# KarelPeeters/kZero

Measured on AMD Instinct MI355X. Metric: self-play NN evals/sec (node), Chess 20x256 ResNet b=256, 1/2/4/8 GPU, higher is better.
Workload: dtype f16; 1 GPU; chess-20x256 attention head, executor batch 256; engines_per_gpu=1, parallelism=dp1 (no collective)

## Files before the change

### kzero_amd/csrc/kz_tower.hip

```cpp
#include <cstdlib>
#include <type_traits>
#include <vector>

#include "kz_kernels.hpp"
#include "kz_launch.hpp"

namespace kz {

typedef _Float16 h16;
typedef h16 h16x8 __attribute__((ext_vector_type(8)));
typedef h16 h16x4 __attribute__((ext_vector_type(4)));
typedef float f32x4 __attribute__((ext_vector_type(4)));

namespace {

#include "kz_decode_dev.hpp"
#include "kz_encode_dev.hpp"

constexpr int C = 256;
constexpr int RS = C * 2 + 16;
constexpr int URS = 3 * C * 2 + 16;
constexpr int KSTEPS = 72;
constexpr int HEAD_KSTEPS = 5 * 8;
constexpr int POLICY = 1880, LOGIT_LD = 96;
constexpr int TOWER_PF_MAX = 8;

struct TowerDev {
    const h16 *x0;
    const uint4 *w_stem, *w_tower;
    const float *bias, *post_scale, *post_shift;
    h16 *y;
    int cin_p, batch, depth;
    PackedBoards in;
    const float *sh_w0, *sh_b0, *sh_w1, *sh_b1, *sh_w2, *sh_b2;
    const int32_t *att_idx;
    float *scalars, *policy;
    int *nonfinite_flag;
    int epoch;
    DecodeDev dec;
};

template <int I, int N, class F>
__device__ __forceinline__ void static_for(F &&f) {
    if constexpr (I < N) {
        f(std::integral_constant<int, I>{});
        static_for<I + 1, N>(f);
    }
}

template <int NB>
struct Layout {
    static constexpr int M = NB * 64;
    static constexpr int MT = M / 16;
    static constexpr bool LINE_TILES = NB == 2;
    static constexpr int BPAD = LINE_TILES ? 128 : 0;
    static constexpr int BOARD = 64 * RS + BPAD;
    static constexpr int TS = LINE_TILES ? 8 * RS : 16 * RS;
    static constexpr int IMG = NB * BOARD;
    static constexpr int X_OFF = 0;
    static constexpr int Y_OFF = IMG;
    static constexpr int Z_OFF = 2 * IMG;
    static_assert(Z_OFF % 256 == 0, "zero rows keep the slot pattern of the image rows");
    static constexpr int S_OFF = Z_OFF + 16 * RS;
    static constexpr int TOWER_BYTES = S_OFF + M * 64;
    static constexpr int U_OFF = Z_OFF;
    static constexpr int ACT_OFF = U_OFF + 16 * URS;
    static constexpr int HID_OFF = ACT_OFF + NB * 256 * 4;
    static constexpr int HEADS_BYTES = HID_OFF + NB * 32 * 4;
    static constexpr int LOG_OFF = Y_OFF;
    static constexpr int BYTES = TOWER_BYTES > HEADS_BYTES ? TOWER_BYTES : HEADS_BYTES;
    static_assert(NB * 64 * LOGIT_LD * 4 <= IMG, "logits fit the Y region");
    static constexpr int row_off(int b, int p) { return b * BOARD + p * RS; }
    static_assert(BYTES <= 160 * 1024, "LDS budget");
};

constexpr int SG_VALU = 0x2, SG_SALU = 0x4, SG_MFMA = 0x8, SG_VMEM_READ = 0x20, SG_DS_READ = 0x100;

template <int NB, bool HEADS, int PF, bool WIDE = false, bool PREV = false>
__global__ __launch_bounds__(256, 1) void kz_tower_resident(TowerDev a) {
    using L = Layout<NB>;
    constexpr int M = L::M, MT = L::MT;
    static_assert(PF <= TOWER_PF_MAX, "the refills past the end of the stream must land in its padding");
    extern __shared__ __attribute__((aligned(16))) unsigned char lds[];

    const int tid = threadIdx.x;
    const int wave = __builtin_amdgcn_readfirstlane(tid >> 6);
    const int lane = tid & 63;
    const int fr = lane & 15, kq = lane >> 4;
    const int board0 = blockIdx.x * NB;
    const int layers = 2 * a.depth;
    const int total_ksteps = layers * KSTEPS + (HEADS ? HEAD_KSTEPS : 0);
    const int bias_rows = layers + (HEADS ? 5 : 0);

    const uint4 *wp = a.w_tower + wave * 256 + lane;
    auto wload_prev = [&](int gk, int nt) __attribute__((always_inline)) { return wp[(size_t)gk * 1024 + nt * 64]; };
    typedef const __attribute__((address_space(1))) unsigned char *gptr;
    gptr wk = (gptr)a.w_tower + wave * 4096;
    const unsigned wlane = lane * 16;
    auto wload = [&](gptr k, int nt) __attribute__((always_inline)) {
        typedef unsigned u32x4 __attribute__((ext_vector_type(4)));
        return __builtin_bit_cast(uint4, *reinterpret_cast<const __attribute__((address_space(1))) u32x4 *>(k + wlane + nt * 1024));
    };
    uint4 wreg[PF][4];
#pragma unroll
    for (int s = 0; s < PF; s++) {
        const int g = s < total_ksteps ? s : total_ksteps - 1;
#pragma unroll
        for (int nt = 0; nt < 4; nt++) wreg[s][nt] = PREV ? wload_prev(g, nt) : wload(wk + s * 16384, nt);
    }
    wk += PF * 16384;
    int g = 0;
    auto ring_take = [&](int stage, h16x8 (&af)[4]) __attribute__((always_inline)) {
#pragma unroll
        for (int nt = 0; nt < 4; nt++) af[nt] = *reinterpret_cast<const h16x8 *>(&wreg[stage][nt]);
#ifndef KZ_TW_NO_WLOAD
        if constexpr (PREV) {
            const int gn = g + PF < total_ksteps ? g + PF : total_ksteps - 1;
#pragma unroll
            for (int nt = 0; nt < 4; nt++) wreg[stage][nt] = wload_prev(gn, nt);
        } else {
#pragma unroll
            for (int nt = 0; nt < 4; nt++) wreg[stage][nt] = wload(wk, nt);
        }
#endif
        wk += 16384;
        if constexpr (!PREV) asm("" : "+s"(wk));
    };

    const int sc = WIDE ? a.cin_p >> 5 : 1;
    const int stem_off = WIDE ? L::Y_OFF : L::S_OFF, srow = 64 * sc, spieces = 4 * sc;
    for (int id = tid; id < 16 * RS / 16; id += 256)
        *reinterpret_cast<uint4 *>(lds + L::Z_OFF + id * 16) = make_uint4(0, 0, 0, 0);
    for (int id = tid; id < M * spieces; id += 256) {
        const int row = WIDE ? id / spieces : id >> 2, c = id - row * spieces;
        const int board = board0 + (row >> 6);
        uint4 v = make_uint4(0, 0, 0, 0);
        if (board < a.batch) {
            if (a.in.bits) {
                h16x8 e;
#pragma unroll
                for (int j = 0; j < 8; j++) e[j] = (h16)encoded_plane(a.in, board, c * 8 + j, row & 63, 64);
                v = *reinterpret_cast<const uint4 *>(&e);
            } else {
                v = *reinterpret_cast<const uint4 *>(a.x0 + ((size_t)board0 * 64 + row) * a.cin_p + c * 8);
            }
        }
        *reinterpret_cast<uint4 *>(lds + stem_off + row * srow + c * 16) = v;
    }
    __syncthreads();

    f32x4 acc[4][MT];
    f32x4 bias_next[4];
    auto fetch_bias = [&](int row) __attribute__((always_inline)) {
        const int l = row <= bias_rows ? row : bias_rows;
#pragma unroll
        for (int nt = 0; nt < 4; nt++)
            bias_next[nt] = *reinterpret_cast<const f32x4 *>(a.bias + l * C + wave * 64 + nt * 16 + kq * 4);
    };
    auto init_acc = [&]() __attribute__((always_inline)) {
#pragma unroll
        for (int nt = 0; nt < 4; nt++)
#pragma unroll
            for (int mt = 0; mt < MT; mt++) acc[nt][mt] = bias_next[nt];
    };
    f32x4 post_s[4], post_t[4];
#pragma unroll
    for (int nt = 0; nt < 4; nt++) {
        post_s[nt] = f32x4{1.f, 1.f, 1.f, 1.f};
        post_t[nt] = f32x4{0.f, 0.f, 0.f, 0.f};
    }

    auto relu4 = [](f32x4 v) {
        typedef int i32x4 __attribute__((ext_vector_type(4)));
        i32x4 b = __builtin_bit_cast(i32x4, v);
#pragma unroll
        for (int j = 0; j < 4; j++) b[j] = b[j] > 0 ? b[j] : 0;
        return __builtin_bit_cast(f32x4, b);
    };
    auto to_h4 = [](f32x4 v) { return h16x4{(h16)v[0], (h16)v[1], (h16)v[2], (h16)v[3]}; };

    const int lane_row = L::LINE_TILES ? (fr >> 3) * L::BOARD + (fr & 7) * RS : fr * RS;
    const int epi_base = lane_row + (wave * 64 + kq * 4) * 2;
    auto epilogue = [&](int dst_off, auto relu, auto residual, auto post) __attribute__((always_inline)) {
#pragma unroll
        for (int nt = 0; nt < 4; nt++) {
            h16x4 rx[MT];
            if constexpr (decltype(residual)::value) {
#pragma unroll
                for (int mt = 0; mt < MT; mt++)
                    rx[mt] = *reinterpret_cast<const h16x4 *>(lds + L::X_OFF + epi_base + mt * L::TS + nt * 32);
            }
#pragma unroll
            for (int mt = 0; mt < MT; mt++) {
                const int off = epi_base + mt * L::TS + nt * 32;
                f32x4 v = acc[nt][mt];
                if constexpr (decltype(relu)::value) v = relu4(v);
                if constexpr (decltype(residual)::value) {
#pragma unroll
                    for (int j = 0; j < 4; j++) v[j] += (float)rx[mt][j];
                }
                if constexpr (decltype(post)::value) v = v * post_s[nt] + post_t[nt];
                *reinterpret_cast<h16x4 *>(lds + dst_off + off) = to_h4(v);
            }
        }
    };
    constexpr std::true_type YES{};
    constexpr std::false_type NO{};

    const bool x_is0 = (lane & 7) == 0, x_is7 = (lane & 7) == 7, yo_is0 = (lane & 8) == 0, yo_is1 = !yo_is0;
    auto tap_ok = [&](int mt, int dy, int dx) __attribute__((always_inline)) {
        const bool kill_x = (dx < 0 && x_is0) || (dx > 0 && x_is7);
        if constexpr (L::LINE_TILES) return !(kill_x || (dy < 0 && mt == 0) || (dy > 0 && mt == MT - 1));
        else return !(kill_x || ((mt & 3) == 0 && dy < 0 && yo_is0) || ((mt & 3) == 3 && dy > 0 && yo_is1));
    };

    fetch_bias(0);
    init_acc();
    fetch_bias(1);
    for (int ks = 0; ks < 9 * sc; ks++) {
        const int tap = WIDE ? ks / sc : ks, chunk = ks - tap * sc;
        const int dy = tap / 3 - 1, dx = tap % 3 - 1;
        h16x8 af[4];
#pragma unroll
        for (int nt = 0; nt < 4; nt++) {
            const uint4 t = a.w_stem[((ks * 4 + wave) * 4 + nt) * 64 + lane];
            af[nt] = *reinterpret_cast<const h16x8 *>(&t);
        }
#pragma unroll
        for (int mt = 0; mt < MT; mt++) {
            const bool ok = tap_ok(mt, dy, dx);
            const int p = L::LINE_TILES ? (fr >> 3) * 64 + mt * 8 + (fr & 7) : mt * 16 + fr;
            const int off = ok ? stem_off + (p + dy * 8 + dx) * srow + chunk * 64 + kq * 16 : L::Z_OFF + kq * 16;
            const h16x8 bf = *reinterpret_cast<const h16x8 *>(lds + off);
#pragma unroll
            for (int nt = 0; nt < 4; nt++)
                acc[nt][mt] = __builtin_amdgcn_mfma_f32_16x16x32_f16(af[nt], bf, acc[nt][mt], 0, 0, 0);
        }
    }
    epilogue(L::X_OFF, NO, NO, NO);
    __syncthreads();

    const int kq_off = 256 * (kq & 1) + 128 * (kq >> 1);
    const int frag_base = lane_row + kq_off;
    auto tap_rows = [&](int dy, int dx, int src_off, int (&T)[MT]) __attribute__((always_inline)) {
        const int shifted = frag_base + src_off + (dy * 8 + dx) * RS;
        const int zrow = L::Z_OFF + ((fr + dy * 8 + dx) & 15) * RS + kq_off;
        const int zrow_odd = L::LINE_TILES ? L::Z_OFF + ((fr + dy * 8 + dx + 8) & 15) * RS + kq_off : zrow;
        if constexpr (PREV) {
#pragma unroll
            for (int mt = 0; mt < MT; mt++) T[mt] = tap_ok(mt, dy, dx) ? shifted + mt * L::TS : ((mt & 1) ? zrow_odd : zrow);
        } else {
            int z0 = zrow, z1 = zrow_odd;
            asm("" : "+v"(z0), "+v"(z1));
            const bool kill_x = ((dx < 0) & x_is0) | ((dx > 0) & x_is7);
#pragma unroll
            for (int mt = 0; mt < MT; mt++) {
                bool kill = kill_x;
                if constexpr (!L::LINE_TILES) kill = kill_x | (((mt & 3) == 0) & (dy < 0) & yo_is0) | (((mt & 3) == 3) & (dy > 0) & yo_is1);
                T[mt] = kill ? ((mt & 1) ? z1 : z0) : shifted + mt * L::TS;
            }
        }
    };

    h16x8 bf[2][MT];
    constexpr auto tile_lo = [](int dy) { return L::LINE_TILES && dy < 0 ? 1 : 0; };
    constexpr auto tile_hi = [](int dy) { return L::LINE_TILES && dy > 0 ? MT - 1 : MT; };

    auto conv_plain = [&](auto ndy_tag, int src_off, int dx_lo, int dx_hi) __attribute__((always_inline)) {
        constexpr int NDY = decltype(ndy_tag)::value, DY0 = NDY == 3 ? -1 : 0;
        int T[NDY][MT], Tn[NDY][MT];
#pragma unroll
        for (int i = 0; i < NDY; i++) tap_rows(DY0 + i, dx_lo, src_off, T[i]);
#pragma unroll
        for (int mt = tile_lo(DY0); mt < tile_hi(DY0); mt++) bf[0][mt] = *reinterpret_cast<const h16x8 *>(lds + T[0][mt]);
#pragma nounroll
        for (int dx = dx_lo; dx < dx_hi; dx++) {
#pragma unroll
            for (int i = 0; i < NDY; i++) tap_rows(DY0 + i, dx + 1 < dx_hi ? dx + 1 : dx, src_off, Tn[i]);
            static_for<0, 8 * NDY>([&](auto s_tag) __attribute__((always_inline)) {
                constexpr int s = decltype(s_tag)::value, ch = s / NDY, i = s % NDY, dy = DY0 + i;
                constexpr int stage = s & (PF - 1), cur = s & 1, nxt = cur ^ 1;
                constexpr int lo = tile_lo(dy), hi = tile_hi(dy), nt_ = hi - lo;
                constexpr int in_ = (i + 1) % NDY, chn = i + 1 < NDY ? ch : ch + 1;
                constexpr int lon = tile_lo(DY0 + in_), hin = tile_hi(DY0 + in_), nr = hin - lon;
#ifndef KZ_TW_NO_DSREAD
#pragma unroll
                for (int mt = 0; mt < MT; mt++) {
                    if (mt >= lon && mt < hin)
                        bf[nxt][mt] = *reinterpret_cast<const h16x8 *>(lds + (chn < 8 ? T[in_][mt] + chn * 16 : Tn[in_][mt]));
                }
#endif
                h16x8 af[4];
                ring_take(stage, af);
#pragma unroll
                for (int nt = 0; nt < 4; nt++)
#pragma unroll
                    for (int mt = 0; mt < MT; mt++)
                        if (mt >= lo && mt < hi)
                            acc[nt][mt] = __builtin_amdgcn_mfma_f32_16x16x32_f16(af[nt], bf[cur][mt], acc[nt][mt], 0, 0, 0);
#pragma unroll
                for (int j = 0; j < 4; j++) {
                    __builtin_amdgcn_sched_group_barrier(SG_MFMA, 1, 0);
                    __builtin_amdgcn_sched_group_barrier(SG_VMEM_READ, 1, 0);
                }
#pragma unroll
                for (int j = 0; j < MT; j++) {
                    if (j < nr) {
                        __builtin_amdgcn_sched_group_barrier(SG_MFMA, 1, 0);
                        __builtin_amdgcn_sched_group_barrier(SG_DS_READ, 1, 0);
                    }
                }
                constexpr int n_free = 4 * nt_ - (nr + 4), n_alu = PREV || s != 0 ? 0 : n_free < 20 ? n_free : 20;
#pragma unroll
                for (int j = 0; j < 20; j++) {
                    if (j < n_alu) {
                        __builtin_amdgcn_sched_group_barrier(SG_MFMA, 1, 0);
                        __builtin_amdgcn_sched_group_barrier(SG_VALU | SG_SALU, 2, 0);
                    }
                }
                __builtin_amdgcn_sched_group_barrier(SG_MFMA, n_free - n_alu, 0);
                __builtin_amdgcn_sched_barrier(0);
                g++;
            });
#pragma unroll
            for (int i = 0; i < NDY; i++)
#pragma unroll
                for (int mt = 0; mt < MT; mt++) T[i][mt] = Tn[i][mt];
        }
    };

    auto conv_3x3_lines = [&](int src_off) __attribute__((always_inline)) {
        static_assert(!L::LINE_TILES || MT == 8, "one tile per board line");
        int T[MT], Tn[MT];
        tap_rows(0, -1, src_off, T);
#pragma unroll
        for (int mt = 0; mt < MT; mt++) bf[0][mt] = *reinterpret_cast<const h16x8 *>(lds + T[mt]);
#pragma nounroll
        for (int dx = -1; dx < 2; dx++) {
            tap_rows(0, dx < 1 ? dx + 1 : dx, src_off, Tn);
            static_for<0, 8>([&](auto ch_tag) __attribute__((always_inline)) {
                constexpr int ch = decltype(ch_tag)::value, cur = ch & 1, nxt = cur ^ 1;
#ifndef KZ_TW_NO_DSREAD
#pragma unroll
                for (int mt = 0; mt < MT; mt++)
                    bf[nxt][mt] = *reinterpret_cast<const h16x8 *>(lds + (ch < 7 ? T[mt] + (ch + 1) * 16 : Tn[mt]));
#endif
                static_for<0, 3>([&](auto i_tag) __attribute__((always_inline)) {
                    constexpr int i = decltype(i_tag)::value, dy = i - 1, stage = (ch * 3 + i) & (PF - 1);
                    constexpr int lo = tile_lo(dy), hi = tile_hi(dy), nt_ = hi - lo;
                    h16x8 af[4];
                    ring_take(stage, af);
#pragma unroll
                    for (int nt = 0; nt < 4; nt++)
#pragma unroll
                        for (int mt = 0; mt < MT; mt++)
                            if (mt >= lo && mt < hi)
                                acc[nt][mt] = __builtin_amdgcn_mfma_f32_16x16x32_f16(af[nt], bf[cur][mt + dy], acc[nt][mt], 0, 0, 0);
#pragma unroll
                    for (int j = 0; j < 4; j++) {
                        __builtin_amdgcn_sched_group_barrier(SG_MFMA, 1, 0);
                        __builtin_amdgcn_sched_group_barrier(SG_VMEM_READ, 1, 0);
                    }
                    constexpr int nr = i == 0 ? MT : 0;
#pragma unroll
                    for (int j = 0; j < MT; j++) {
                        if (j < nr) {
                            __builtin_amdgcn_sched_group_barrier(SG_MFMA, 1, 0);
                            __builtin_amdgcn_sched_group_barrier(SG_DS_READ, 1, 0);
                        }
                    }
                    constexpr int n_free = 4 * nt_ - (nr + 4), n_alu = ch == 0 && i == 0 ? n_free : 0;
#pragma unroll
                    for (int j = 0; j < 4 * MT; j++) {
                        if (j < n_alu) {
                            __builtin_amdgcn_sched_group_barrier(SG_MFMA, 1, 0);
                            __builtin_amdgcn_sched_group_barrier(SG_VALU | SG_SALU, 2, 0);
                        }
                    }
                    __builtin_amdgcn_sched_group_barrier(SG_MFMA, n_free - n_alu, 0);
                    __builtin_amdgcn_sched_barrier(0);
                    g++;
                });
            });
#pragma unroll
            for (int mt = 0; mt < MT; mt++) T[mt] = Tn[mt];
        }
    };
    constexpr std::integral_constant<int, 3> THREE_ROWS{};
    constexpr std::integral_constant<int, 1> ONE_ROW{};
    auto conv_3x3 = [&](int src_off) __attribute__((always_inline)) {
        if constexpr (L::LINE_TILES && !PREV) conv_3x3_lines(src_off);
        else conv_plain(THREE_ROWS, src_off, -1, 2);
    };
    auto conv_1x1 = [&](int src_off) __attribute__((always_inline)) { conv_plain(ONE_ROW, src_off, 0, 1); };

    for (int layer = 1; layer <= layers; layer++) {
        const bool is_b = (layer & 1) == 0;
        init_acc();
        fetch_bias(layer + 1);
        if (layer == layers) {
#pragma unroll
            for (int nt = 0; nt < 4; nt++) {
                const int oc = wave * 64 + nt * 16 + kq * 4;
                post_s[nt] = *reinterpret_cast<const f32x4 *>(a.post_scale + oc);
                post_t[nt] = *reinterpret_cast<const f32x4 *>(a.post_shift + oc);
            }
        }
        conv_3x3(is_b ? L::Y_OFF : L::X_OFF);
        if (!is_b) epilogue(L::Y_OFF, YES, NO, NO);
        else if (layer != layers) epilogue(L::X_OFF, YES, YES, NO);
        else epilogue(L::X_OFF, YES, YES, YES);
        __syncthreads();
    }

    if constexpr (!HEADS) {
        for (int id = tid; id < M * 32; id += 256) {
            const int p = id >> 5, c16 = id & 31;
            const int board = board0 + (p >> 6);
            if (board < a.batch) {
                const uint4 v = *reinterpret_cast<const uint4 *>(lds + L::X_OFF + L::row_off(p >> 6, p & 63) + c16 * 16);
                *reinterpret_cast<uint4 *>(a.y + ((size_t)board0 * 64 + p) * C + c16 * 8) = v;
            }
        }
    } else {
        {
            float *act = reinterpret_cast<float *>(lds + L::ACT_OFF);
            for (int o = tid; o < NB * 256; o += 256) {
                const int b = o >> 8, c4 = (o >> 6) & 3, p = o & 63;
                const unsigned char *row = lds + L::X_OFF + L::row_off(b, p);
                const float *w = a.sh_w0 + c4 * C;
                float s = a.sh_b0[c4];
#pragma unroll 4
                for (int i = 0; i < C; i += 8) {
                    const h16x8 xv = *reinterpret_cast<const h16x8 *>(row + i * 2);
                    const f32x4 w0 = *reinterpret_cast<const f32x4 *>(w + i), w1 = *reinterpret_cast<const f32x4 *>(w + i + 4);
#pragma unroll
                    for (int j = 0; j < 4; j++) s += (float)xv[j] * w0[j] + (float)xv[4 + j] * w1[j];
                }
                if (!(fabsf(s) <= 3.0e38f) && a.nonfinite_flag && board0 + b < a.batch) {
                    *reinterpret_cast<volatile int *>(a.nonfinite_flag) = a.epoch;
                    raise_nonfinite_board(a.nonfinite_flag, a.epoch, board0 + b);
                }
                act[o] = fmaxf(s, 0.0f);
            }
        }

        {
            const int tb = L::X_OFF + L::row_off(NB == 2 ? fr >> 3 : 0, 56 + (fr & 7)) + kq_off;
            for (int s = 0; s < 3; s++) {
                f32x4 ua[4];
#pragma unroll
                for (int nt = 0; nt < 4; nt++) ua[nt] = bias_next[nt];
                fetch_bias(layers + 2 + s);
#pragma unroll
                for (int ch = 0; ch < 8; ch++) {
                    const h16x8 bf = *reinterpret_cast<const h16x8 *>(lds + tb + ch * 16);
                    h16x8 af[4];
                    ring_take(ch & (PF - 1), af);
#pragma unroll
                    for (int nt = 0; nt < 4; nt++)
                        ua[nt] = __builtin_amdgcn_mfma_f32_16x16x32_f16(af[nt], bf, ua[nt], 0, 0, 0);
                    g++;
                }
                if (NB == 2 || fr < 8) {
#pragma unroll
                    for (int nt = 0; nt < 4; nt++)
                        *reinterpret_cast<h16x4 *>(lds + L::U_OFF + fr * URS + (256 * s + wave * 64 + nt * 16 + kq * 4) * 2) =
                            to_h4(ua[nt]);
                }
            }
        }

        init_acc();
        fetch_bias(layers + 5);
        conv_1x1(L::X_OFF);
        epilogue(L::Y_OFF, NO, NO, NO);

        init_acc();
        conv_1x1(L::X_OFF);
        __syncthreads();
        epilogue(L::X_OFF, NO, NO, NO);
        __syncthreads();

        {
            const float *act = reinterpret_cast<const float *>(lds + L::ACT_OFF);
            float *hid = reinterpret_cast<float *>(lds + L::HID_OFF);
            if (tid < NB * 128) {
                const int pair = tid >> 2, part = tid & 3, b = pair >> 5, j = pair & 31;
                const float *w = a.sh_w1 + j * 256 + part * 64;
                const float *x = act + b * 256 + part * 64;
                float s = 0.0f;
#pragma unroll 4
                for (int i = 0; i < 64; i += 4) {
                    const f32x4 wv = *reinterpret_cast<const f32x4 *>(w + i), xv = *reinterpret_cast<const f32x4 *>(x + i);
                    s += wv[0] * xv[0] + wv[1] * xv[1] + wv[2] * xv[2] + wv[3] * xv[3];
                }
                s += __shfl_xor(s, 1, 64);
                s += __shfl_xor(s, 2, 64);
                if (part == 0) hid[b * 32 + j] = fmaxf(s + a.sh_b1[j], 0.0f);
            }
        }

        constexpr int IT = NB == 2 ? 2 : 1;
        const int hb = NB == 2 ? wave >> 1 : 0;
        const int it0 = NB == 2 ? (wave & 1) * 2 : wave;
        f32x4 la[IT][6];
        {
            int ja[6], ia[IT];
#pragma unroll
            for (int jt = 0; jt < 4; jt++) ja[jt] = L::X_OFF + L::row_off(hb, jt * 16 + fr) + kq_off;
            ja[4] = L::U_OFF + (hb * 8 + (fr & 7)) * URS + (fr >> 3) * 512 + kq_off;
            ja[5] = L::U_OFF + (hb * 8 + (fr & 7)) * URS + 2 * 512 + kq_off;
#pragma unroll
            for (int ii = 0; ii < IT; ii++) ia[ii] = L::Y_OFF + L::row_off(hb, (it0 + ii) * 16 + fr) + kq_off;
#pragma unroll
            for (int ii = 0; ii < IT; ii++)
#pragma unroll
                for (int jt = 0; jt < 6; jt++) la[ii][jt] = f32x4{0.f, 0.f, 0.f, 0.f};
#pragma unroll
            for (int ch = 0; ch < 8; ch++) {
                h16x8 qa[6], qb[IT];
#pragma unroll
                for (int jt = 0; jt < 6; jt++) qa[jt] = *reinterpret_cast<const h16x8 *>(lds + ja[jt] + ch * 16);
#pragma unroll
                for (int ii = 0; ii < IT; ii++) qb[ii] = *reinterpret_cast<const h16x8 *>(lds + ia[ii] + ch * 16);
#pragma unroll
                for (int ii = 0; ii < IT; ii++)
#pragma unroll
                    for (int jt = 0; jt < 6; jt++)
                        la[ii][jt] = __builtin_amdgcn_mfma_f32_16x16x32_f16(qa[jt], qb[ii], la[ii][jt], 0, 0, 0);
            }
        }
        __syncthreads();
        {
            const float inv = 1.0f / sqrtf((float)C);
#pragma unroll
            for (int ii = 0; ii < IT; ii++)
#pragma unroll
                for (int jt = 0; jt < 6; jt++) {
                    const int i = (it0 + ii) * 16 + fr, j = jt * 16 + kq * 4;
                    *reinterpret_cast<f32x4 *>(lds + L::LOG_OFF + ((hb * 64 + i) * LOGIT_LD + j) * 4) = la[ii][jt] * inv;
                }
        }
        const bool decode = a.dec.move_offsets != nullptr;
        float *raw = reinterpret_cast<float *>(lds + L::ACT_OFF);
        if (tid < NB * 5) {
            const int b = tid / 5, k = tid % 5;
            const float *hid = reinterpret_cast<const float *>(lds + L::HID_OFF) + b * 32;
            float s = a.sh_b2[k];
            for (int i = 0; i < 32; i++) s += a.sh_w2[k * 32 + i] * hid[i];
            if (decode) raw[b * 8 + k] = s;
            else if (board0 + b < a.batch) a.scalars[(size_t)(board0 + b) * 5 + k] = s;
        }
        __syncthreads();
        if (decode) {
            if (wave < NB && board0 + wave < a.batch) {
                const float *lg = reinterpret_cast<const float *>(lds + L::LOG_OFF) + wave * 64 * LOGIT_LD;
                float *stage = reinterpret_cast<float *>(lds + L::X_OFF + L::row_off(wave, 0));
                decode_board_wave(a.dec, board0 + wave, lane, raw + wave * 8, stage, 64 * RS / 4,
                                  [&](int idx) { return lg[a.att_idx[idx]]; });
            }
        } else {
            for (int b = 0; b < NB; b++) {
                if (board0 + b >= a.batch) break;
                const float *lg = reinterpret_cast<const float *>(lds + L::LOG_OFF) + b * 64 * LOGIT_LD;
                float *pol = a.policy + (size_t)(board0 + b) * POLICY;
                for (int k = tid; k < POLICY; k += 256) pol[k] = lg[a.att_idx[k]];
            }
        }
    }
}

#ifndef KZ_PF_NB1
#define KZ_PF_NB1 4
#endif
#ifndef KZ_PF_NB2
#define KZ_PF_NB2 4
#endif
constexpr int PF_NB1 = KZ_PF_NB1, PF_NB2 = KZ_PF_NB2;

void pack_1x1(const float *w, uint16_t *dst) {
    static const int kq_base[4] = {0, 128, 64, 192};
    for (int chunk = 0; chunk < 8; chunk++)
        for (int wave = 0; wave < 4; wave++)
            for (int nt = 0; nt < 4; nt++)
                for (int lane = 0; lane < 64; lane++)
                    for (int j = 0; j < 8; j++) {
                        const int oc = 64 * wave + 16 * nt + (lane & 15);
                        const int ch = 8 * chunk + kq_base[lane >> 4] + j;
                        const _Float16 hv = (_Float16)w[(size_t)oc * 256 + ch];
                        uint16_t bits;
                        __builtin_memcpy(&bits, &hv, 2);
                        dst[((((size_t)chunk * 4 + wave) * 4 + nt) * 64 + lane) * 8 + j] = bits;
                    }
}

}

bool tower_resident_supported(int dtype, int h, int w, int channels, int depth, int c_in) {
    return dtype == 1 && h == 8 && w == 8 && channels == C && depth >= 1 && c_in >= 1 && c_in <= 224;
}

bool tower_heads_supported(int policy_kind, int query_channels, int policy_len, int sh_channels, int sh_size) {
    return policy_kind == 2 && query_channels == C && policy_len == POLICY && sh_channels == 4 && sh_size == 32;
}

size_t tower_packed_weight_elems(int cin_p, int depth) {
    return (size_t)9 * C * cin_p + (size_t)2 * depth * 9 * C * C;
}

size_t tower_heads_weight_elems() { return (size_t)HEAD_KSTEPS * 16 * 1024 / 2; }

size_t tower_weight_pad_elems() { return (size_t)TOWER_PF_MAX * 16 * 1024 / 2; }

void tower_pack_weights(const float *oihw, int cout, int cin, int cin_p, uint16_t *dst, bool tap_major) {
    const int nchunk = cin_p / 32;
    const bool rows_inner = cin_p == 256 && !tap_major;
    static const int kq_base[4] = {0, 128, 64, 192};
    for (int tap = 0; tap < 9; tap++)
        for (int chunk = 0; chunk < nchunk; chunk++) {
            const size_t kstep = rows_inner ? ((size_t)(tap % 3) * 8 + chunk) * 3 + tap / 3 : (size_t)tap * nchunk + chunk;
            for (int wave = 0; wave < 4; wave++)
                for (int nt = 0; nt < 4; nt++)
                    for (int lane = 0; lane < 64; lane++)
                        for (int j = 0; j < 8; j++) {
                            const int oc = 64 * wave + 16 * nt + (lane & 15);
                            const int kq = lane >> 4;
                            const int ch = cin_p == 256 ? 8 * chunk + kq_base[kq] + j : 32 * chunk + 8 * kq + j;
                            float v = 0.0f;
                            if (oc < cout && ch < cin) v = oihw[((size_t)oc * cin + ch) * 9 + tap];
                            const _Float16 hv = (_Float16)v;
                            uint16_t bits;
                            __builtin_memcpy(&bits, &hv, 2);
                            dst[(((kstep * 4 + wave) * 4 + nt) * 64 + lane) * 8 + j] = bits;
                        }
        }
}

void tower_pack_heads(const float *w_bulk , const float *b_bulk, const float *w_under ,
                      const float *b_under, uint16_t *dst, float *bias5) {
    const size_t pass = (size_t)8 * 16 * 1024 / 2;
    std::vector<float> tmp((size_t)256 * 256);
    for (int s = 0; s < 3; s++) {
        for (int q = 0; q < 256; q++) {
            for (int c = 0; c < 256; c++) tmp[(size_t)q * 256 + c] = w_under[(size_t)(3 * q + s) * 256 + c];
            bias5[s * 256 + q] = b_under[3 * q + s];
        }
        pack_1x1(tmp.data(), dst + pass * s);
    }
    pack_1x1(w_bulk, dst + pass * 3);
    pack_1x1(w_bulk + (size_t)256 * 256, dst + pass * 4);
    for (int q = 0; q < 256; q++) {
        bias5[3 * 256 + q] = b_bulk[q];
        bias5[4 * 256 + q] = b_bulk[256 + q];
    }
}

namespace {
template <auto Kernel>
void launch_instance(const TowerDev &d, int grid, int bytes, hipStream_t stream) {
    allow_dynamic_lds<Kernel>(bytes);
    Kernel<<<grid, 256, bytes, stream>>>(d);
}
}

void launch_tower_resident(const TowerArgs &t, hipStream_t stream) {
    TowerDev d{};
    d.x0 = static_cast<const h16 *>(t.x0);
    d.w_stem = static_cast<const uint4 *>(t.w_stem);
    d.w_tower = static_cast<const uint4 *>(t.w_tower);
    d.bias = t.bias;
    d.post_scale = t.post_scale;
    d.post_shift = t.post_shift;
    d.y = static_cast<h16 *>(t.y);
    d.cin_p = t.cin_p;
    d.batch = t.batch;
    d.depth = t.depth;
    d.in = t.in;
    d.sh_w0 = t.sh_w0; d.sh_b0 = t.sh_b0; d.sh_w1 = t.sh_w1; d.sh_b1 = t.sh_b1; d.sh_w2 = t.sh_w2; d.sh_b2 = t.sh_b2;
    d.att_idx = t.att_idx;
    d.scalars = t.scalars;
    d.policy = t.policy;
    d.nonfinite_flag = t.nonfinite_flag;
    d.epoch = t.epoch;
    d.dec = decode_dev(t.decode, t.fused_heads, POLICY);
    const bool heads = t.fused_heads;
#ifdef KZ_EXPERIMENTS
    if (t.prev) {
        const int grid = (t.batch + 1) / 2;
        if (t.cin_p > 32) {
            if (heads) launch_instance<kz_tower_resident<2, true, PF_NB2, true, true>>(d, grid, Layout<2>::BYTES, stream);
            else launch_instance<kz_tower_resident<2, false, PF_NB2, true, true>>(d, grid, Layout<2>::BYTES, stream);
        } else if (t.boards_per_wg == 1) {
            if (heads) launch_instance<kz_tower_resident<1, true, PF_NB1, false, true>>(d, t.batch, Layout<1>::BYTES, stream);
            else launch_instance<kz_tower_resident<1, false, PF_NB1, false, true>>(d, t.batch, Layout<1>::BYTES, stream);
        } else {
            if (heads) launch_instance<kz_tower_resident<2, true, PF_NB2, false, true>>(d, grid, Layout<2>::BYTES, stream);
            else launch_instance<kz_tower_resident<2, false, PF_NB2, false, true>>(d, grid, Layout<2>::BYTES, stream);
        }
        return;
    }
#endif
    if (t.cin_p > 32) {
        const int grid = (t.batch + 1) / 2;
        if (heads) launch_instance<kz_tower_resident<2, true, PF_NB2, true>>(d, grid, Layout<2>::BYTES, stream);
        else launch_instance<kz_tower_resident<2, false, PF_NB2, true>>(d, grid, Layout<2>::BYTES, stream);
    } else if (t.boards_per_wg == 1) {
        if (heads) launch_instance<kz_tower_resident<1, true, PF_NB1>>(d, t.batch, Layout<1>::BYTES, stream);
        else launch_instance<kz_tower_resident<1, false, PF_NB1>>(d, t.batch, Layout<1>::BYTES, stream);
    } else {
        const int grid = (t.batch + 1) / 2;
        if (heads) launch_instance<kz_tower_resident<2, true, PF_NB2>>(d, grid, Layout<2>::BYTES, stream);
        else launch_instance<kz_tower_resident<2, false, PF_NB2>>(d, grid, Layout<2>::BYTES, stream);
    }
}

}
```

Measured before the change: 551,700 evals/s.

## Fold bias init into first MFMA and overlap ReLU with final conv MFMAs

Measured after the change: 556,900 evals/s (median of 6 runs). About the same (+0.9%).

```diff
diff --git a/kzero_amd/csrc/kz_tower.hip b/kzero_amd/csrc/kz_tower.hip
--- a/kzero_amd/csrc/kz_tower.hip
+++ b/kzero_amd/csrc/kz_tower.hip
@@ -178,10 +178,21 @@
         return __builtin_bit_cast(f32x4, b);
     };
     auto to_h4 = [](f32x4 v) { return h16x4{(h16)v[0], (h16)v[1], (h16)v[2], (h16)v[3]}; };
+    auto relu_h4 = [](h16x4 h) {
+        typedef short i16x4 __attribute__((ext_vector_type(4)));
+        i16x4 b = __builtin_bit_cast(i16x4, h);
+#pragma unroll
+        for (int j = 0; j < 4; j++) b[j] = b[j] > 0 ? b[j] : (short)0;
+        return __builtin_bit_cast(h16x4, b);
+    };
+    constexpr bool LINES = L::LINE_TILES && !PREV;
+    constexpr int N0_EARLY = 7;
 
     const int lane_row = L::LINE_TILES ? (fr >> 3) * L::BOARD + (fr & 7) * RS : fr * RS;
     const int epi_base = lane_row + (wave * 64 + kq * 4) * 2;
-    auto epilogue = [&](int dst_off, auto relu, auto residual, auto post) __attribute__((always_inline)) {
+    constexpr auto leaves_early = [](int n0, int nt, int mt) { return n0 >= 0 && (mt == MT - 1 || (nt == 0 && mt < n0)); };
+    auto epilogue = [&](int dst_off, auto relu, auto residual, auto post, auto n0_tag) __attribute__((always_inline)) {
+        constexpr int N0 = decltype(n0_tag)::value;
 #pragma unroll
         for (int nt = 0; nt < 4; nt++) {
             h16x4 rx[MT];
@@ -194,7 +205,12 @@
             for (int mt = 0; mt < MT; mt++) {
                 const int off = epi_base + mt * L::TS + nt * 32;
                 f32x4 v = acc[nt][mt];
-                if constexpr (decltype(relu)::value) v = relu4(v);
+                const bool relu_done = leaves_early(N0, nt, mt);
+                if constexpr (LINES && decltype(relu)::value && !decltype(residual)::value && !decltype(post)::value) {
+                    *reinterpret_cast<h16x4 *>(lds + dst_off + off) = relu_done ? to_h4(v) : relu_h4(to_h4(v));
+                    continue;
+                }
+                if (decltype(relu)::value && !relu_done) v = relu4(v);
                 if constexpr (decltype(residual)::value) {
 #pragma unroll
                     for (int j = 0; j < 4; j++) v[j] += (float)rx[mt][j];
@@ -204,6 +220,7 @@
             }
         }
     };
+    constexpr std::integral_constant<int, -1> ALL_TILES{};
     constexpr std::true_type YES{};
     constexpr std::false_type NO{};
 
@@ -237,7 +254,7 @@
                 acc[nt][mt] = __builtin_amdgcn_mfma_f32_16x16x32_f16(af[nt], bf, acc[nt][mt], 0, 0, 0);
         }
     }
-    epilogue(L::X_OFF, NO, NO, NO);
+    epilogue(L::X_OFF, NO, NO, NO, ALL_TILES);
     __syncthreads();
 
     const int kq_off = 256 * (kq & 1) + 128 * (kq >> 1);
@@ -329,39 +346,48 @@
         }
     };
 
-    auto conv_3x3_lines = [&](int src_off) __attribute__((always_inline)) {
+    auto conv_3x3_lines = [&](int src_off, int bias_row) __attribute__((always_inline)) {
         static_assert(!L::LINE_TILES || MT == 8, "one tile per board line");
         int T[MT], Tn[MT];
         tap_rows(0, -1, src_off, T);
 #pragma unroll
         for (int mt = 0; mt < MT; mt++) bf[0][mt] = *reinterpret_cast<const h16x8 *>(lds + T[mt]);
-#pragma nounroll
-        for (int dx = -1; dx < 2; dx++) {
-            tap_rows(0, dx < 1 ? dx + 1 : dx, src_off, Tn);
+        auto dx_body = [&](auto dx_tag) __attribute__((always_inline)) {
+            constexpr int dx = decltype(dx_tag)::value;
+            constexpr bool FIRST = dx == -1;
+            if constexpr (dx < 1) tap_rows(0, dx + 1, src_off, Tn);
             static_for<0, 8>([&](auto ch_tag) __attribute__((always_inline)) {
                 constexpr int ch = decltype(ch_tag)::value, cur = ch & 1, nxt = cur ^ 1;
+                constexpr bool LAST = dx == 1 && ch == 7;
 #ifndef KZ_TW_NO_DSREAD
-#pragma unroll
-                for (int mt = 0; mt < MT; mt++)
-                    bf[nxt][mt] = *reinterpret_cast<const h16x8 *>(lds + (ch < 7 ? T[mt] + (ch + 1) * 16 : Tn[mt]));
+                if constexpr (!LAST) {
+#pragma unroll
+                    for (int mt = 0; mt < MT; mt++)
+                        bf[nxt][mt] = *reinterpret_cast<const h16x8 *>(lds + (ch < 7 ? T[mt] + (ch + 1) * 16 : Tn[mt]));
+                }
 #endif
                 static_for<0, 3>([&](auto i_tag) __attribute__((always_inline)) {
                     constexpr int i = decltype(i_tag)::value, dy = i - 1, stage = (ch * 3 + i) & (PF - 1);
                     constexpr int lo = tile_lo(dy), hi = tile_hi(dy), nt_ = hi - lo;
                     h16x8 af[4];
                     ring_take(stage, af);
+                    constexpr int nb = FIRST && ch == 0 && i == 2 ? 4 : 0;
+                    if constexpr (nb != 0) fetch_bias(bias_row);
 #pragma unroll
                     for (int nt = 0; nt < 4; nt++)
 #pragma unroll
                         for (int mt = 0; mt < MT; mt++)
-                            if (mt >= lo && mt < hi)
-                                acc[nt][mt] = __builtin_amdgcn_mfma_f32_16x16x32_f16(af[nt], bf[cur][mt + dy], acc[nt][mt], 0, 0, 0);
-#pragma unroll
-                    for (int j = 0; j < 4; j++) {
+                            if (mt >= lo && mt < hi) {
+                                const bool first_touch = FIRST && ch == 0 && (i == 0 || (i == 1 && mt == 0));
+                                acc[nt][mt] = __builtin_amdgcn_mfma_f32_16x16x32_f16(af[nt], bf[cur][mt + dy],
+                                                                                   first_touch ? bias_next[nt] : acc[nt][mt], 0, 0, 0);
+                            }
+#pragma unroll
+                    for (int j = 0; j < 4 + nb; j++) {
                         __builtin_amdgcn_sched_group_barrier(SG_MFMA, 1, 0);
                         __builtin_amdgcn_sched_group_barrier(SG_VMEM_READ, 1, 0);
                     }
-                    constexpr int nr = i == 0 ? MT : 0;
+                    constexpr int nr = i == 0 && !LAST ? MT : 0;
 #pragma unroll
                     for (int j = 0; j < MT; j++) {
                         if (j < nr) {
@@ -369,35 +395,57 @@
                             __builtin_amdgcn_sched_group_barrier(SG_DS_READ, 1, 0);
                         }
                     }
-                    constexpr int n_free = 4 * nt_ - (nr + 4), n_alu = ch == 0 && i == 0 ? n_free : 0;
-#pragma unroll
-                    for (int j = 0; j < 4 * MT; j++) {
-                        if (j < n_alu) {
+                    constexpr int n_free = 4 * nt_ - (nr + 4 + nb);
+                    if constexpr (LAST && i == 2) {
+#pragma unroll
+                        for (int nt = 0; nt < 4; nt++)
+#pragma unroll
+                            for (int mt = 0; mt < MT; mt++)
+                                if (leaves_early(N0_EARLY, nt, mt)) acc[nt][mt] = relu4(acc[nt][mt]);
+#pragma unroll
+                        for (int j = 0; j < n_free; j++) {
                             __builtin_amdgcn_sched_group_barrier(SG_MFMA, 1, 0);
-                            __builtin_amdgcn_sched_group_barrier(SG_VALU | SG_SALU, 2, 0);
+                            __builtin_amdgcn_sched_group_barrier(SG_VALU, 4, 0);
                         }
+                    } else {
+                        constexpr int n_alu = ch == 0 && i == 0 ? n_free : 0;
+#pragma unroll
+                        for (int j = 0; j < 4 * MT; j++) {
+                            if (j < n_alu) {
+                                __builtin_amdgcn_sched_group_barrier(SG_MFMA, 1, 0);
+                                __builtin_amdgcn_sched_group_barrier(SG_VALU | SG_SALU, 2, 0);
+                            }
+                        }
+                        __builtin_amdgcn_sched_group_barrier(SG_MFMA, n_free - n_alu, 0);
                     }
-                    __builtin_amdgcn_sched_group_barrier(SG_MFMA, n_free - n_alu, 0);
                     __builtin_amdgcn_sched_barrier(0);
                     g++;
                 });
             });
-#pragma unroll
-            for (int mt = 0; mt < MT; mt++) T[mt] = Tn[mt];
-        }
+            if constexpr (dx < 1) {
+#pragma unroll
+                for (int mt = 0; mt < MT; mt++) T[mt] = Tn[mt];
+            }
+        };
+        dx_body(std::integral_constant<int, -1>{});
+        dx_body(std::integral_constant<int, 0>{});
+        dx_body(std::integral_constant<int, 1>{});
     };
     constexpr std::integral_constant<int, 3> THREE_ROWS{};
     constexpr std::integral_constant<int, 1> ONE_ROW{};
-    auto conv_3x3 = [&](int src_off) __attribute__((always_inline)) {
-        if constexpr (L::LINE_TILES && !PREV) conv_3x3_lines(src_off);
-        else conv_plain(THREE_ROWS, src_off, -1, 2);
+    auto conv_3x3 = [&](int src_off, int bias_row) __attribute__((always_inline)) {
+        if constexpr (LINES) {
+            conv_3x3_lines(src_off, bias_row);
+        } else {
+            init_acc();
+            fetch_bias(bias_row);
+            conv_plain(THREE_ROWS, src_off, -1, 2);
+        }
     };
     auto conv_1x1 = [&](int src_off) __attribute__((always_inline)) { conv_plain(ONE_ROW, src_off, 0, 1); };
 
     for (int layer = 1; layer <= layers; layer++) {
         const bool is_b = (layer & 1) == 0;
-        init_acc();
-        fetch_bias(layer + 1);
         if (layer == layers) {
 #pragma unroll
             for (int nt = 0; nt < 4; nt++) {
@@ -406,10 +454,11 @@
                 post_t[nt] = *reinterpret_cast<const f32x4 *>(a.post_shift + oc);
             }
         }
-        conv_3x3(is_b ? L::Y_OFF : L::X_OFF);
-        if (!is_b) epilogue(L::Y_OFF, YES, NO, NO);
-        else if (layer != layers) epilogue(L::X_OFF, YES, YES, NO);
-        else epilogue(L::X_OFF, YES, YES, YES);
+        conv_3x3(is_b ? L::Y_OFF : L::X_OFF, layer + 1);
+        constexpr std::integral_constant<int, LINES ? N0_EARLY : -1> EARLY{};
+        if (!is_b) epilogue(L::Y_OFF, YES, NO, NO, EARLY);
+        else if (layer != layers) epilogue(L::X_OFF, YES, YES, NO, EARLY);
+        else epilogue(L::X_OFF, YES, YES, YES, EARLY);
         __syncthreads();
     }
 
@@ -474,12 +523,12 @@
         init_acc();
         fetch_bias(layers + 5);
         conv_1x1(L::X_OFF);
-        epilogue(L::Y_OFF, NO, NO, NO);
+        epilogue(L::Y_OFF, NO, NO, NO, ALL_TILES);
 
         init_acc();
         conv_1x1(L::X_OFF);
         __syncthreads();
-        epilogue(L::X_OFF, NO, NO, NO);
+        epilogue(L::X_OFF, NO, NO, NO, ALL_TILES);
         __syncthreads();
 
         {
```
